# KhutornoyYaroslav/vcm-ts

Hardware: AMD Instinct MI355X
Metric: encoded frames/sec at 1920x1080 GOP-32 (higher is better)
Workload: dtype f32 (fp16x3 split-MFMA, fp32 accumulate)

## Files before the change

include/dcvc_hip.h:

```cpp
#ifndef DCVC_HIP_H
#define DCVC_HIP_H

#include <stdint.h>

#ifdef __cplusplus
extern "C" {
#endif

#define DCVC_OK 0
#define DCVC_E_ARG (-1)
#define DCVC_E_LAUNCH (-2)
#define DCVC_E_RANGE (-3)

#define DCVC_STATUS_ACT_SATURATED 1

#define DCVC_MAX_SEG 3

#define DCVC_PREC_FP32 0
#define DCVC_PREC_FP16X3 1

typedef struct {
    const float *ptr;
    int32_t C;
    int32_t cs;
} dcvc_seg;

typedef struct {
    dcvc_seg seg[DCVC_MAX_SEG];
    int32_t nseg;
    int32_t N, Hin, Win;
    int32_t in_act;
    float in_slope;
    const float *wpack;
    const float *bpack;
    int32_t ks;
    int32_t stride;
    int32_t Cout;
    int32_t Cout_pad;
    float *out;
    int32_t out_cs;
    int32_t out_act;
    float out_slope;
    int32_t pixel_shuffle;
    const float *res;
    int32_t res_cs;
    const float *res_gate;
    const float *res2;
    int32_t res2_cs;
    int32_t precision;
    int32_t *status;
    float *chan_partial;
    int32_t tile_row0;
    int32_t tile_rows;
    int32_t pair_taps;
} dcvc_conv_args;

int32_t dcvc_conv_tile_rows(int32_t ks, int32_t stride);

int32_t dcvc_conv_chan_partial_parts(int32_t ks, int32_t stride, int32_t Hout, int32_t Wout);
int dcvc_channel_mean_finish(const float *chan_partial, int32_t parts, int32_t row_stride, float *mean, int32_t N,
                             int32_t C, int32_t HW, void *stream);

int64_t dcvc_conv_pack_size(int32_t Cout, int32_t ks, int32_t nseg, const int32_t *seg_C, int32_t *cout_pad);

int dcvc_conv_pack_weights(const float *w, const float *b, int32_t Cout, int32_t ks, int32_t nseg,
                           const int32_t *seg_C, int32_t pixel_shuffle, int32_t precision, float *wpack,
                           float *bpack);

int64_t dcvc_conv_pack_size_paired(int32_t Cout, int32_t Cin, int32_t *cout_pad);
int dcvc_conv_pack_weights_paired(const float *w, const float *b, int32_t Cout, int32_t Cin, float *wpack, float *bpack);

int dcvc_conv2d(const dcvc_conv_args *a, void *stream);

int64_t dcvc_conv_small_pack_bytes(int32_t Cout, int32_t ks, int32_t nseg, const int32_t *seg_C);
int dcvc_conv_small_pack_weights(const float *w, const float *b, int32_t Cout, int32_t ks, int32_t nseg,
                                 const int32_t *seg_C, void *wpack, float *bpack);
int dcvc_conv2d_small(const dcvc_conv_args *a, void *stream);

int64_t dcvc_conv_k32_pack_bytes(int32_t Cout, int32_t ks, int32_t nseg, const int32_t *seg_C, int32_t *cout_pad);
int dcvc_conv_k32_pack_weights(const float *w, const float *b, int32_t Cout, int32_t ks, int32_t nseg,
                               const int32_t *seg_C, int32_t pixel_shuffle, void *wpack, float *bpack);
int dcvc_conv2d_k32(const dcvc_conv_args *a, void *stream);
int dcvc_conv_k32_set_waves(int32_t waves);

int dcvc_warp(const float *src, int32_t src_cs, const float *flow, int32_t flow_cs, float *out, int32_t out_cs,
              int32_t N, int32_t H, int32_t W, int32_t C, void *stream);
int dcvc_up2(const float *src, int32_t src_cs, float *out, int32_t out_cs, float *out2, int32_t out2_cs,
             int32_t N, int32_t H, int32_t W, int32_t C, float scale, void *stream);
int dcvc_down2(const float *src, int32_t src_cs, float *out, int32_t out_cs, int32_t N, int32_t H, int32_t W,
               int32_t C, float scale, int32_t avgpool_order, void *stream);
int dcvc_maxpool2(const float *src, int32_t src_cs, float *out, int32_t out_cs, int32_t N, int32_t H, int32_t W,
                  int32_t C, void *stream);
int dcvc_copy_channels(const float *src, int32_t src_cs, float *out, int32_t out_cs, int64_t npix, int32_t C,
                       void *stream);
int dcvc_nchw_to_nhwc(const float *src, float *out, int32_t out_cs, int32_t N, int32_t C, int32_t H, int32_t W,
                      void *stream);
int dcvc_nhwc_to_nchw(const float *src, int32_t src_cs, float *out, int32_t N, int32_t C, int32_t H, int32_t W,
                      int32_t clamp01, void *stream);

int dcvc_channel_mean(const float *src, int32_t src_cs, float *mean, float *scratch, int32_t N, int32_t HW,
                      int32_t C, void *stream);
int dcvc_se_gate(const float *mean, const float *w1, const float *w2, float *gate, int32_t N, int32_t C,
                 int32_t Cr, void *stream);

int dcvc_scale_channels(const float *src, int32_t src_cs, float *out, int32_t out_cs, const float *q_basic,
                        const float *q_scale, int32_t mode, int32_t N, int32_t HW, int32_t C, void *stream);
int dcvc_scale_channels_map(const float *src, int32_t src_cs, float *out, int32_t out_cs, const float *q_basic,
                            const float *q_scale, int32_t mode, int32_t N, int32_t HW, int32_t C, const float *q_map,
                            int32_t H, int32_t W, void *stream);
int dcvc_round_symbols(const float *z, int32_t z_cs, float *z_hat, int32_t zh_cs, int32_t *sym, int32_t N,
                       int32_t H, int32_t W, int32_t C, void *stream);
int dcvc_symbols_to_nhwc(const int32_t *sym, float *out, int32_t out_cs, int32_t N, int32_t H, int32_t W,
                         int32_t C, void *stream);

typedef struct {
    const float *y;
    int32_t y_cs;
    const float *fusion;
    int32_t fusion_cs;
    const float *spatial;
    int32_t spatial_cs;
    float *params;
    int32_t params_cs;
    float *y_hat;
    float *y_q;
    float *y_res;
    float *scales_hat;
    int32_t *sym;
    int32_t *idx;
    float *out;
    int32_t out_cs;
    const float *q_basic;
    const float *q_scale;
    int32_t N, H, W, C;
    int32_t step;
    const float *idx_edges;
    const float *forced_q;
    const float *q_map;
} dcvc_dual_prior_args;

int dcvc_scale_indexes(const float *scales, int32_t *idx, int64_t n, const float *idx_edges, void *stream);

int dcvc_dual_prior_enc(const dcvc_dual_prior_args *a, void *stream);
int dcvc_dual_prior_dec_index(const dcvc_dual_prior_args *a, void *stream);
int dcvc_dual_prior_dec_apply(const dcvc_dual_prior_args *a, void *stream);

int dcvc_scale_bits(const float *y_q, const float *scales_hat, float *out, float *scratch, int32_t kind, int32_t N,
                    int64_t per_sample, void *stream);
int dcvc_factorized_bits(const float *z_hat, int32_t z_cs, const float *params, float *out, float *scratch, int32_t N,
                         int32_t HW, int32_t C, void *stream);
int dcvc_sq_err(const float *a, int32_t a_cs, const float *b, int32_t b_cs, float *out, float *scratch, int32_t N,
                int32_t HW, int32_t C, void *stream);

int32_t dcvc_cdf_table_cols(void);
int dcvc_build_scale_cdfs(const float *scales, int32_t n_scales, int32_t kind, int32_t *cdf, int32_t *sizes,
                          int32_t *offsets, void *stream);
int dcvc_build_factorized_cdfs(const float *params, int32_t C, int32_t *cdf, int32_t *sizes, int32_t *offsets, void *stream);

const char *dcvc_hip_version(void);

#ifdef __cplusplus
}
#endif
#endif
```

vcm_ts_amd/csrc/conv_mfma.hip:

```cpp
#include <hip/hip_runtime.h>
#include <stdint.h>
#include <stdlib.h>
#include <string.h>
#include <vector>

#include "dcvc_hip.h"
#include "kernel_common.h"

namespace {

constexpr int LDK = 20;


struct ConvK {
    const float *seg_ptr[DCVC_MAX_SEG];
    int seg_C[DCVC_MAX_SEG];
    int seg_cs[DCVC_MAX_SEG];
    int nseg;
    int Hin, Win, Hout, Wout;
    int in_act;
    float in_slope;
    const float *wpack;
    const float *bpack;
    int Cout, Cout_pad;
    float *out;
    int out_cs;
    int out_act;
    float out_slope;
    int ps;
    const float *res;
    int res_cs;
    const float *res_gate;
    const float *res2;
    int res2_cs;
    int vec_epi;
    int *status;
    float *chan_partial;
    int ntx;
    int ty0, nty;
    int band_rows;
};

inline long dev_env_long(const char *name, long dflt) {
    const char *dev = getenv("DCVC_DEV");
    if (!dev || strcmp(dev, "1") != 0) return dflt;
    const char *v = getenv(name);
    return v ? atol(v) : dflt;
}


template <int KS, int S, int RPW, int NT, bool SPLIT, bool PAIR = false>
__global__ __launch_bounds__(256, 2) void conv_mfma(const ConvK a) {
    static_assert(!PAIR || (KS == 7 && S == 1 && SPLIT), "tap pairing is built for the 7x7 split-fp16 layers");
    constexpr int BH = 4 * RPW, BW = 32, BN = 32 * NT;
    constexpr int PH = (BH - 1) * S + KS, PW = (BW - 1) * S + KS, PAD = KS / 2;
    constexpr int T = PAIR ? KS * 4 : KS * KS;
    constexpr int TPS = PAIR ? 4 : (KS == 3 && S == 1) ? 9 : KS;
    constexpr int NST = T / TPS;
    constexpr int EPI_LD = BN + 4;
    constexpr int LDS_MAIN = PH * PW * LDK + TPS * 4 * BN * 4, LDS_EPI = 4 * 32 * EPI_LD, LDS_RED = 4 * BN;
    __shared__ __attribute__((aligned(16))) float lds[LDS_MAIN > LDS_EPI + LDS_RED ? LDS_MAIN : LDS_EPI + LDS_RED];
    float *patch = lds;
    float *wl = lds + PH * PW * LDK;

    const int tid = threadIdx.x, lane = tid & 63, wave = tid >> 6;
    const int nbn = a.Cout_pad / BN;
    const int nb = blockIdx.x % nbn, tx = blockIdx.x / nbn;
    if (tx >= a.ntx) return;
    const int ty = blockIdx.y + a.ty0;
    const int x0 = tx * BW, y0 = ty * BH, n0 = nb * BN, img = blockIdx.z;

    f32x16 acc[RPW][NT];
#pragma unroll
    for (int m = 0; m < RPW; ++m)
#pragma unroll
        for (int n = 0; n < NT; ++n)
#pragma unroll
            for (int r = 0; r < 16; ++r) acc[m][n][r] = 0.f;

    const int a_base = ((wave * RPW * S) * PW + (lane & 31) * S) * LDK + (lane >> 5) * 4;
    const int b_base = ((lane >> 5) * BN + (lane & 31)) * 4;

    constexpr int NP = (PH * PW * 4 + 255) / 256, NW = (TPS * 4 * BN + 255) / 256;
    f32x4 rp[NP], rw[NW];
    struct Cursor {
        int s, c0, cg, st;
    };
    auto advance = [&](Cursor &k) {
        if (++k.st == NST) {
            k.st = 0;
            ++k.cg;
            k.c0 += MFMA_KC;
            if (k.c0 >= a.seg_C[k.s]) {
                ++k.s;
                k.c0 = 0;
            }
        }
    };
    int poff[NP];
    unsigned inpic = 0;
#pragma unroll
    for (int u = 0; u < NP; ++u) {
        const int i = tid + u * 256;
        const int p = i >> 2;
        const int py = p / PW, px = p - py * PW + (PAIR ? (i & 3) >> 1 : 0);
        const int gy = y0 * S - PAD + py, gx = x0 * S - PAD + px;
        const bool ok = i < PH * PW * 4 && gy >= 0 && gy < a.Hin && gx >= 0 && gx < a.Win;
        poff[u] = ok ? gy * a.Win + gx : 0;
        inpic |= (ok ? 1u : 0u) << u;
    }
    auto load_patch = [&](const Cursor &k) {
        const int C = a.seg_C[k.s], cs = a.seg_cs[k.s];
        const float *sp = a.seg_ptr[k.s] + (size_t)img * a.Hin * a.Win * cs;
        const int c = PAIR ? (tid & 1) * 4 : k.c0 + (tid & 3) * 4;
        const int cc = c < C ? c : 0;
#pragma unroll
        for (int u = 0; u < NP; ++u) rp[u] = *(const f32x4 *)(sp + (size_t)poff[u] * cs + cc);
    };
    auto store_patch = [&](const Cursor &k) {
        const int C = a.seg_C[k.s];
#pragma unroll
        for (int u = 0; u < NP; ++u) {
            const int i = tid + u * 256;
            if (i < PH * PW * 4) {
                const int c = PAIR ? (i & 1) * 4 : k.c0 + (i & 3) * 4;
                f32x4 v = ((inpic >> u) & 1u) && c < C ? rp[u] : (f32x4){0.f, 0.f, 0.f, 0.f};
                if (c + 3 >= C) {
                    if (c + 1 >= C) v[1] = 0.f;
                    if (c + 2 >= C) v[2] = 0.f;
                    v[3] = 0.f;
                }
                if (a.in_act) {
                    v[0] = act(v[0], a.in_slope);
                    v[1] = act(v[1], a.in_slope);
                    v[2] = act(v[2], a.in_slope);
                    v[3] = act(v[3], a.in_slope);
                }
                if (!SPLIT) {
                    *(f32x4 *)&patch[(i >> 2) * LDK + (i & 3) * 4] = v;
                } else {
                    f32x4 sv = v * ACT_SCALE;
#pragma unroll
                    for (int e = 0; e < 4; ++e) sv[e] = __builtin_amdgcn_fmed3f(sv[e], -F16_MAX, F16_MAX);
                    const f16x4 hi = __builtin_convertvector(sv, f16x4);
                    const f16x4 lo = __builtin_convertvector(sv - __builtin_convertvector(hi, f32x4), f16x4);
                    _Float16 *rec = (_Float16 *)&patch[(i >> 2) * LDK];
                    *(f16x4 *)&rec[(i & 3) * 4] = hi;
                    *(f16x4 *)&rec[16 + (i & 3) * 4] = lo;
                }
            }
        }
    };
    auto load_w = [&](const Cursor &k) {
        const float *wsrc = a.wpack + ((size_t)(k.cg * T + k.st * TPS) * 4) * a.Cout_pad * 4 + (size_t)n0 * 4;
#pragma unroll
        for (int u = 0; u < NW; ++u) {
            const int i = tid + u * 256;
            const int row = i / BN, col = i - row * BN;
            if (i < TPS * 4 * BN) rw[u] = *(const f32x4 *)(wsrc + ((size_t)row * a.Cout_pad + col) * 4);
        }
    };
    auto store_w = [&]() {
#pragma unroll
        for (int u = 0; u < NW; ++u) {
            const int i = tid + u * 256;
            if (i < TPS * 4 * BN) *(f32x4 *)&wl[i * 4] = rw[u];
        }
    };

    Cursor cur = {0, 0, 0, 0};
    load_patch(cur);
    load_w(cur);
    while (cur.s < a.nseg) {
        __syncthreads();
        if (cur.st == 0) store_patch(cur);
        store_w();
        __syncthreads();
        Cursor nxt = cur;
        advance(nxt);
        if (nxt.s < a.nseg) {
            if (nxt.st == 0) load_patch(nxt);
            load_w(nxt);
        }
        const int a_st = (TPS == T) ? 0 : cur.st * PW * LDK;
#pragma unroll
        for (int tt = 0; tt < TPS; ++tt) {
            const int ky = (TPS == T) ? tt / KS : 0, kx = PAIR ? 2 * tt : (TPS == T) ? tt % KS : tt;
            if (!SPLIT) {
#pragma unroll
                for (int k2 = 0; k2 < 2; ++k2) {
                    f32x4 af[RPW], bf[NT];
#pragma unroll
                    for (int m = 0; m < RPW; ++m)
                        af[m] = *(const f32x4 *)&patch[a_base + a_st + ((m * S + ky) * PW + kx) * LDK + k2 * 8];
#pragma unroll
                    for (int n = 0; n < NT; ++n)
                        bf[n] = *(const f32x4 *)&wl[b_base + ((tt * 4 + k2 * 2) * BN + n * 32) * 4];
#pragma unroll
                    for (int j = 0; j < 4; ++j)
#pragma unroll
                        for (int m = 0; m < RPW; ++m)
#pragma unroll
                            for (int n = 0; n < NT; ++n)
                                acc[m][n] = __builtin_amdgcn_mfma_f32_32x32x2f32(af[m][j], bf[n][j], acc[m][n], 0, 0, 0);
                }
            } else {
                f16x8 ah[RPW], al[RPW], bh[NT], bl[NT];
#pragma unroll
                for (int m = 0; m < RPW; ++m) {
                    const float *rec = &patch[a_base + a_st + ((m * S + ky) * PW + kx) * LDK];
                    ah[m] = *(const f16x8 *)rec;
                    al[m] = *(const f16x8 *)(rec + 8);
                }
#pragma unroll
                for (int n = 0; n < NT; ++n) {
                    bh[n] = *(const f16x8 *)&wl[b_base + ((tt * 4) * BN + n * 32) * 4];
                    bl[n] = *(const f16x8 *)&wl[b_base + ((tt * 4 + 2) * BN + n * 32) * 4];
                }
#pragma unroll
                for (int m = 0; m < RPW; ++m)
#pragma unroll
                    for (int n = 0; n < NT; ++n) {
                        acc[m][n] = __builtin_amdgcn_mfma_f32_32x32x16_f16(ah[m], bh[n], acc[m][n], 0, 0, 0);
                        acc[m][n] = __builtin_amdgcn_mfma_f32_32x32x16_f16(ah[m], bl[n], acc[m][n], 0, 0, 0);
                        acc[m][n] = __builtin_amdgcn_mfma_f32_32x32x16_f16(al[m], bh[n], acc[m][n], 0, 0, 0);
                    }
            }
        }
        cur = nxt;
    }

    const int col = lane & 31, hh = lane >> 5;
    const int Cq = a.Cout >> 2;
    const int Cfin = a.ps ? Cq : a.Cout;
    const int Ho = a.ps ? a.Hout * 2 : a.Hout, Wo = a.ps ? a.Wout * 2 : a.Wout;
    const float inv_scale = SPLIT ? 1.f / (ACT_SCALE * WGT_SCALE) : 1.f;
    float vmax = 0.f;
    if (a.vec_epi) {
        constexpr int LPP = BN / 4, PPI = 64 / LPP, NIT = 32 / PPI;
        float *epi = lds + wave * 32 * EPI_LD;
        const int c4 = (lane % LPP) * 4, pl = lane / LPP;
        const int ch = n0 + c4;
        const bool ch_ok = ch < a.Cout;
        int dy = 0, dx = 0, cf = ch;
        if (a.ps) {
            const int sub = ch / Cq;
            cf = ch - sub * Cq;
            dy = sub >> 1;
            dx = sub & 1;
        }
        f32x4 bias = {0.f, 0.f, 0.f, 0.f}, gate = {1.f, 1.f, 1.f, 1.f};
        if (ch_ok) {
            bias = *(const f32x4 *)&a.bpack[ch];
            if (a.res_gate) gate = *(const f32x4 *)&a.res_gate[(size_t)img * Cfin + cf];
        }
        __syncthreads();
        size_t pix[RPW][NIT];
        bool ok[RPW][NIT];
        f32x4 rv[RPW][NIT], rv2[RPW][NIT];
        f32x4 csum = {0.f, 0.f, 0.f, 0.f};
#pragma unroll
        for (int m = 0; m < RPW; ++m) {
            const int oy = y0 + wave * RPW + m;
#pragma unroll
            for (int it = 0; it < NIT; ++it) {
                const int ox = x0 + it * PPI + pl;
                ok[m][it] = ch_ok && oy < a.Hout && ox < a.Wout;
                pix[m][it] = a.ps ? ((size_t)(img * Ho + 2 * oy + dy) * Wo + 2 * ox + dx) : ((size_t)(img * Ho + oy) * Wo + ox);
                rv[m][it] = (f32x4){0.f, 0.f, 0.f, 0.f};
                rv2[m][it] = (f32x4){0.f, 0.f, 0.f, 0.f};
                if (ok[m][it] && a.res) rv[m][it] = *(const f32x4 *)&a.res[pix[m][it] * a.res_cs + cf];
                if (ok[m][it] && a.res2) rv2[m][it] = *(const f32x4 *)&a.res2[pix[m][it] * a.res2_cs + cf];
            }
        }
#pragma unroll
        for (int m = 0; m < RPW; ++m) {
#pragma unroll
            for (int n = 0; n < NT; ++n)
#pragma unroll
                for (int r = 0; r < 16; ++r)
                    epi[((r & 3) + 8 * (r >> 2) + 4 * hh) * EPI_LD + n * 32 + col] = acc[m][n][r];
            asm volatile("s_waitcnt lgkmcnt(0)" ::: "memory");
#pragma unroll
            for (int it = 0; it < NIT; ++it) {
                f32x4 v = *(const f32x4 *)&epi[(it * PPI + pl) * EPI_LD + c4];
                v = v * inv_scale + bias;
                if (a.out_act == 1) {
                    v[0] = act(v[0], a.out_slope);
                    v[1] = act(v[1], a.out_slope);
                    v[2] = act(v[2], a.out_slope);
                    v[3] = act(v[3], a.out_slope);
                } else if (a.out_act == 2) {
#pragma unroll
                    for (int e = 0; e < 4; ++e) v[e] = fminf(fmaxf(v[e], 0.f), 1.f);
                }
                if (a.out_act == 3) {
#pragma unroll
                    for (int e = 0; e < 4; ++e) {
                        const float mk = rv2[m][it][e] > 0.f ? 1.f : a.out_slope;
                        v[e] = a.res ? __builtin_fmaf(v[e], mk, rv[m][it][e]) : v[e] * mk;
                    }
                } else {
                    if (a.res) {
                        if (a.res_gate) {
#pragma unroll
                            for (int e = 0; e < 4; ++e) v[e] = __builtin_fmaf(rv[m][it][e], gate[e], v[e]);
                        } else {
                            v = v + rv[m][it];
                        }
                    }
                    if (a.res2) v = rv2[m][it] + v;
                }
                if (a.chan_partial && ok[m][it]) csum += v;
                if (a.status && ok[m][it])
                    vmax = fmaxf(vmax, fmaxf(fmaxf(fabsf(v[0]), fabsf(v[1])), fmaxf(fabsf(v[2]), fabsf(v[3]))));
                if (ok[m][it]) *(f32x4 *)&a.out[pix[m][it] * a.out_cs + cf] = v;
            }
            asm volatile("s_waitcnt lgkmcnt(0)" ::: "memory");
        }
        if (a.status && !(vmax <= ACT_LIMIT)) atomicOr(a.status, DCVC_STATUS_ACT_SATURATED);
        if (a.chan_partial) {
#pragma unroll
            for (int off = LPP; off < 64; off <<= 1)
#pragma unroll
                for (int e = 0; e < 4; ++e) csum[e] += __shfl_xor(csum[e], off);
            float *red = lds + LDS_EPI;
            if (lane < LPP) *(f32x4 *)&red[wave * BN + c4] = csum;
            __syncthreads();
            if (tid < BN && n0 + tid < a.Cout_pad) {
                const float s = ((red[tid] + red[BN + tid]) + red[2 * BN + tid]) + red[3 * BN + tid];
                const size_t part = (size_t)img * (a.nty * a.ntx) + (size_t)ty * a.ntx + tx;
                a.chan_partial[part * a.Cout_pad + n0 + tid] = s;
            }
        }
        return;
    }
#pragma unroll
    for (int m = 0; m < RPW; ++m) {
        const int oy = y0 + wave * RPW + m;
        if (oy >= a.Hout) continue;
#pragma unroll
        for (int n = 0; n < NT; ++n) {
            const int ch = n0 + n * 32 + col;
            if (ch >= a.Cout) continue;
            const float bias = a.bpack[ch];
            int dy = 0, dx = 0, cf = ch;
            if (a.ps) {
                const int sub = ch / Cq;
                cf = ch - sub * Cq;
                dy = sub >> 1;
                dx = sub & 1;
            }
            const float gate = a.res_gate ? a.res_gate[(size_t)img * Cfin + cf] : 1.f;
            float rv[16], rv2[16];
#pragma unroll
            for (int r = 0; r < 16; ++r) {
                const int ox = x0 + (r & 3) + 8 * (r >> 2) + 4 * hh;
                const size_t pix = a.ps ? ((size_t)(img * Ho + 2 * oy + dy) * Wo + 2 * ox + dx)
                                        : ((size_t)(img * Ho + oy) * Wo + ox);
                rv[r] = (a.res && ox < a.Wout) ? a.res[pix * a.res_cs + cf] : 0.f;
                rv2[r] = (a.res2 && ox < a.Wout) ? a.res2[pix * a.res2_cs + cf] : 0.f;
            }
#pragma unroll
            for (int r = 0; r < 16; ++r) {
                const int ox = x0 + (r & 3) + 8 * (r >> 2) + 4 * hh;
                if (ox >= a.Wout) continue;
                float v = acc[m][n][r] * inv_scale + bias;
                if (a.out_act == 1) v = act(v, a.out_slope);
                else if (a.out_act == 2) v = fminf(fmaxf(v, 0.f), 1.f);
                const size_t pix = a.ps ? ((size_t)(img * Ho + 2 * oy + dy) * Wo + 2 * ox + dx)
                                        : ((size_t)(img * Ho + oy) * Wo + ox);
                if (a.out_act == 3) {
                    const float mk = rv2[r] > 0.f ? 1.f : a.out_slope;
                    v = a.res ? __builtin_fmaf(v, mk, rv[r]) : v * mk;
                } else {
                    if (a.res) v = a.res_gate ? __builtin_fmaf(rv[r], gate, v) : v + rv[r];
                    if (a.res2) v = rv2[r] + v;
                }
                if (a.status) vmax = fmaxf(vmax, fabsf(v));
                a.out[pix * a.out_cs + cf] = v;
            }
        }
    }
    if (a.status && !(vmax <= ACT_LIMIT)) atomicOr(a.status, DCVC_STATUS_ACT_SATURATED);
}


template <int KS, int S, int RPW, int NT, bool PAIR = false>
int launch(ConvK &k, int N, hipStream_t st, int precision) {
    constexpr int BH = 4 * RPW, BN = 32 * NT;
    k.ntx = (k.Wout + 31) / 32;
    static const bool xcd_pad = dev_env_long("DCVC_XCD_PAD", 0) != 0;
    unsigned gx = (unsigned)(k.ntx * (k.Cout_pad / BN));
    if (xcd_pad && gx >= 8) gx = (gx + 7) & ~7u;
    k.nty = (k.Hout + BH - 1) / BH;
    if (k.ty0 < 0 || k.ty0 >= k.nty) return DCVC_E_ARG;
    const int rows = k.band_rows > 0 ? (k.band_rows < k.nty - k.ty0 ? k.band_rows : k.nty - k.ty0) : k.nty;
    dim3 grid(gx, (unsigned)rows, (unsigned)N);
    if (PAIR)
        hipLaunchKernelGGL((conv_mfma<KS, S, RPW, NT, true, PAIR>), grid, dim3(256), 0, st, k);
    else if (precision == DCVC_PREC_FP16X3)
        hipLaunchKernelGGL((conv_mfma<KS, S, RPW, NT, true>), grid, dim3(256), 0, st, k);
    else
        hipLaunchKernelGGL((conv_mfma<KS, S, RPW, NT, false>), grid, dim3(256), 0, st, k);
    RET_LAUNCH();
}

}

extern "C" int64_t dcvc_conv_pack_size(int32_t Cout, int32_t ks, int32_t nseg, const int32_t *seg_C, int32_t *cout_pad) {
    if (Cout <= 0 || nseg <= 0 || nseg > DCVC_MAX_SEG || (ks != 1 && ks != 3 && ks != 7)) return DCVC_E_ARG;
    int chunks = 0;
    for (int s = 0; s < nseg; ++s) chunks += (seg_C[s] + MFMA_KC - 1) / MFMA_KC;
    const int cp = round_up(Cout, 32);
    if (cout_pad) *cout_pad = cp;
    return (int64_t)chunks * ks * ks * 4 * cp * 4;
}

extern "C" int dcvc_conv_pack_weights(const float *w, const float *b, int32_t Cout, int32_t ks, int32_t nseg,
                                      const int32_t *seg_C, int32_t pixel_shuffle, int32_t precision, float *wpack,
                                      float *bpack) {
    if (precision != DCVC_PREC_FP32 && precision != DCVC_PREC_FP16X3) return DCVC_E_ARG;
    int32_t cp = 0;
    const int64_t total = dcvc_conv_pack_size(Cout, ks, nseg, seg_C, &cp);
    if (total < 0 || (pixel_shuffle && (Cout & 3))) return DCVC_E_ARG;
    const int T = ks * ks;
    int Cin = 0;
    for (int s = 0; s < nseg; ++s) Cin += seg_C[s];
    memset(wpack, 0, (size_t)total * sizeof(float));
    memset(bpack, 0, (size_t)cp * sizeof(float));
    const int Cq = Cout / 4;
    _Float16 *base = (_Float16 *)wpack;
    int cg = 0, cin0 = 0;
    for (int s = 0; s < nseg; ++s) {
        for (int c0 = 0; c0 < seg_C[s]; c0 += MFMA_KC, ++cg) {
            for (int t = 0; t < T; ++t)
                for (int cc = 0; cc < MFMA_KC && c0 + cc < seg_C[s]; ++cc)
                    for (int n = 0; n < Cout; ++n) {
                        const int np = pixel_shuffle ? ps_packed_channel(n, Cq) : n;
                        const float v = w[((size_t)n * Cin + cin0 + c0 + cc) * T + t];
                        if (precision == DCVC_PREC_FP32) {
                            wpack[mfma_wpack_f32(cg, T, t, cc, cp, np)] = v;
                        } else {
                            float sv = v * WGT_SCALE;
                            sv = sv > F16_MAX ? F16_MAX : (sv < -F16_MAX ? -F16_MAX : sv);
                            const SplitF16 p = split_f16(sv);
                            base[mfma_wpack_f16(cg, T, t, cc, cp, np, 0)] = p.hi;
                            base[mfma_wpack_f16(cg, T, t, cc, cp, np, 1)] = p.lo;
                        }
                    }
        }
        cin0 += seg_C[s];
    }
    for (int n = 0; n < Cout; ++n) bpack[pixel_shuffle ? ps_packed_channel(n, Cq) : n] = b ? b[n] : 0.f;
    return DCVC_OK;
}

extern "C" int64_t dcvc_conv_pack_size_paired(int32_t Cout, int32_t Cin, int32_t *cout_pad) {
    if (Cout <= 0 || Cin <= 0 || Cin > 8) return DCVC_E_ARG;
    const int cp = round_up(Cout, 32);
    if (cout_pad) *cout_pad = cp;
    return (int64_t)7 * 4 * 4 * cp * 4;
}

extern "C" int dcvc_conv_pack_weights_paired(const float *w, const float *b, int32_t Cout, int32_t Cin, float *wpack, float *bpack) {
    int32_t cp = 0;
    const int64_t total = dcvc_conv_pack_size_paired(Cout, Cin, &cp);
    if (total < 0 || !w || !wpack || !bpack) return DCVC_E_ARG;
    memset(wpack, 0, (size_t)total * sizeof(float));
    memset(bpack, 0, (size_t)cp * sizeof(float));
    _Float16 *base = (_Float16 *)wpack;
    bool clamped = false;
    for (int ky = 0; ky < 7; ++ky)
        for (int kx = 0; kx < 7; ++kx) {
            const int step = ky * 4 + (kx >> 1), h = kx & 1;
            for (int c = 0; c < Cin; ++c)
                for (int n = 0; n < Cout; ++n) {
                    float sv = w[((size_t)n * Cin + c) * 49 + ky * 7 + kx] * WGT_SCALE;
                    if (!(fabsf(sv) <= F16_MAX)) { clamped = true; sv = sv > 0.f ? F16_MAX : -F16_MAX; }
                    const SplitF16 p = split_f16(sv);
                    base[mfma_wpack_f16(0, 28, step, 8 * h + c, cp, n, 0)] = p.hi;
                    base[mfma_wpack_f16(0, 28, step, 8 * h + c, cp, n, 1)] = p.lo;
                }
        }
    for (int n = 0; n < Cout; ++n) bpack[n] = b ? b[n] : 0.f;
    return clamped ? DCVC_E_RANGE : DCVC_OK;
}

static int tile_rows(int ks, int stride) { return stride == 2 ? 4 : 8; }

extern "C" int32_t dcvc_conv_tile_rows(int32_t ks, int32_t stride) { return tile_rows(ks, stride); }

extern "C" int32_t dcvc_conv_chan_partial_parts(int32_t ks, int32_t stride, int32_t Hout, int32_t Wout) {
    if (Hout <= 0 || Wout <= 0 || (stride != 1 && stride != 2)) return DCVC_E_ARG;
    const int bh = tile_rows(ks, stride);
    return ((Wout + 31) / 32) * ((Hout + bh - 1) / bh);
}

extern "C" int dcvc_conv2d(const dcvc_conv_args *a, void *stream) {
    if (!conv_args_ok(a)) return DCVC_E_ARG;
    if (a->stride != 1 && a->stride != 2) return DCVC_E_ARG;
    if (a->precision != DCVC_PREC_FP32 && a->precision != DCVC_PREC_FP16X3) return DCVC_E_ARG;
    if (a->Cout_pad % 32 || a->Cout > a->Cout_pad || (a->pixel_shuffle && (a->Cout & 3))) return DCVC_E_ARG;
    if (a->out_act < 0 || a->out_act > 3) return DCVC_E_ARG;
    if (a->out_act == 3 && (!a->res2 || a->res_gate || a->chan_partial || a->pixel_shuffle)) return DCVC_E_ARG;
    ConvK k;
    memset(&k, 0, sizeof(k));
    copy_conv_args_full(k, a);
    k.Hin = a->Hin;
    k.Win = a->Win;
    const int pad = a->ks / 2;
    k.Hout = (a->Hin + 2 * pad - a->ks) / a->stride + 1;
    k.Wout = (a->Win + 2 * pad - a->ks) / a->stride + 1;
    k.vec_epi = vec_epilogue_ok(a);
    if (a->chan_partial && (!k.vec_epi || a->pixel_shuffle)) return DCVC_E_ARG;
    hipStream_t st = (hipStream_t)stream;
    const bool wide = (a->Cout_pad % 64) == 0;
    const int key = a->ks * 10 + a->stride;
    if (a->stride == 1 && !a->pair_taps && !a->chan_partial && a->tile_rows <= 0) {
        const long wgs8 = (long)((k.Wout + 31) / 32) * ((k.Hout + 7) / 8) * (a->Cout_pad / (wide ? 64 : 32)) * a->N;
        static const long rows4_below = dev_env_long("DCVC_ROWS4_WGS", 384);
        if (wgs8 < rows4_below) {
            if (a->ks == 3) return wide ? launch<3, 1, 1, 2>(k, a->N, st, a->precision) : launch<3, 1, 1, 1>(k, a->N, st, a->precision);
            if (a->ks == 7) return wide ? launch<7, 1, 1, 2>(k, a->N, st, a->precision) : launch<7, 1, 1, 1>(k, a->N, st, a->precision);
            if (a->ks == 1) return wide ? launch<1, 1, 1, 2>(k, a->N, st, a->precision) : launch<1, 1, 1, 1>(k, a->N, st, a->precision);
        }
    }
    switch (key) {
        case 11: return wide ? launch<1, 1, 2, 2>(k, a->N, st, a->precision) : launch<1, 1, 2, 1>(k, a->N, st, a->precision);
        case 12: return wide ? launch<1, 2, 1, 2>(k, a->N, st, a->precision) : launch<1, 2, 1, 1>(k, a->N, st, a->precision);
        case 31:
            return wide ? launch<3, 1, 2, 2>(k, a->N, st, a->precision) : launch<3, 1, 2, 1>(k, a->N, st, a->precision);
        case 32: return wide ? launch<3, 2, 1, 2>(k, a->N, st, a->precision) : launch<3, 2, 1, 1>(k, a->N, st, a->precision);
        case 71:
            if (a->pair_taps) {
                if (a->nseg != 1 || a->seg[0].C > 8 || a->precision != DCVC_PREC_FP16X3 || a->pixel_shuffle) return DCVC_E_ARG;
                return wide ? launch<7, 1, 2, 2, true>(k, a->N, st, a->precision) : launch<7, 1, 2, 1, true>(k, a->N, st, a->precision);
            }
            return wide ? launch<7, 1, 2, 2>(k, a->N, st, a->precision) : launch<7, 1, 2, 1>(k, a->N, st, a->precision);
        default: return DCVC_E_ARG;
    }
}
```

vcm_ts_amd/lib.py:

```python
from __future__ import annotations

import ctypes as C
import os

HERE = os.path.dirname(os.path.abspath(__file__))
CSRC = os.path.join(HERE, "csrc")


class LibraryMissing(RuntimeError):
    pass


class KernelError(RuntimeError):
    pass


def _load(name):
    path = os.environ.get("DCVC_HIP_LIB") if name == "libdcvc_hip.so" and os.environ.get("DCVC_HIP_LIB") else \
        os.path.join(CSRC, name)
    if not os.path.exists(path):
        raise LibraryMissing(f"{path} not built; run `make -C {CSRC}` (no CPU fallback exists)")
    return C.CDLL(path)


_rans = None


def rans():
    global _rans
    if _rans is None:
        L = _load("libdcvc_rans.so")
        L.dcvc_rans_encoder_create.restype = C.c_void_p
        L.dcvc_rans_encoder_destroy.argtypes = [C.c_void_p]
        L.dcvc_rans_encoder_reset.argtypes = [C.c_void_p]
        L.dcvc_rans_encoder_encode_with_indexes.argtypes = [C.c_void_p, C.c_void_p, C.c_void_p, C.c_int64, C.c_void_p,
                                                            C.c_int32, C.c_int32, C.c_void_p, C.c_void_p]
        L.dcvc_rans_encoder_flush_bound.argtypes = [C.c_void_p]
        L.dcvc_rans_encoder_flush_bound.restype = C.c_int64
        L.dcvc_rans_encoder_flush.argtypes = [C.c_void_p, C.c_void_p, C.c_int64]
        L.dcvc_rans_encoder_flush.restype = C.c_int64
        L.dcvc_rans_decoder_create.restype = C.c_void_p
        L.dcvc_rans_decoder_destroy.argtypes = [C.c_void_p]
        L.dcvc_rans_decoder_set_stream.argtypes = [C.c_void_p, C.c_char_p, C.c_int64]
        L.dcvc_rans_decoder_decode_stream.argtypes = [C.c_void_p, C.c_void_p, C.c_int64, C.c_void_p, C.c_int32,
                                                      C.c_int32, C.c_void_p, C.c_void_p, C.c_void_p]
        L.dcvc_pmf_to_quantized_cdf.argtypes = [C.c_void_p, C.c_int32, C.c_int32, C.c_void_p]
        _rans = L
    return _rans


class Seg(C.Structure):
    _fields_ = [("ptr", C.c_void_p), ("C", C.c_int32), ("cs", C.c_int32)]


class ConvArgs(C.Structure):
    _fields_ = [
        ("seg", Seg * 3), ("nseg", C.c_int32), ("N", C.c_int32), ("Hin", C.c_int32), ("Win", C.c_int32),
        ("in_act", C.c_int32), ("in_slope", C.c_float), ("wpack", C.c_void_p), ("bpack", C.c_void_p),
        ("ks", C.c_int32), ("stride", C.c_int32), ("Cout", C.c_int32), ("Cout_pad", C.c_int32),
        ("out", C.c_void_p), ("out_cs", C.c_int32), ("out_act", C.c_int32), ("out_slope", C.c_float),
        ("pixel_shuffle", C.c_int32), ("res", C.c_void_p), ("res_cs", C.c_int32), ("res_gate", C.c_void_p),
        ("res2", C.c_void_p), ("res2_cs", C.c_int32), ("precision", C.c_int32), ("status", C.c_void_p),
        ("chan_partial", C.c_void_p), ("tile_row0", C.c_int32), ("tile_rows", C.c_int32), ("pair_taps", C.c_int32),
    ]


class DualPriorArgs(C.Structure):
    _fields_ = [
        ("y", C.c_void_p), ("y_cs", C.c_int32), ("fusion", C.c_void_p), ("fusion_cs", C.c_int32),
        ("spatial", C.c_void_p), ("spatial_cs", C.c_int32), ("params", C.c_void_p), ("params_cs", C.c_int32),
        ("y_hat", C.c_void_p), ("y_q", C.c_void_p), ("y_res", C.c_void_p), ("scales_hat", C.c_void_p),
        ("sym", C.c_void_p), ("idx", C.c_void_p), ("out", C.c_void_p), ("out_cs", C.c_int32),
        ("q_basic", C.c_void_p), ("q_scale", C.c_void_p), ("N", C.c_int32), ("H", C.c_int32), ("W", C.c_int32),
        ("C", C.c_int32), ("step", C.c_int32), ("idx_edges", C.c_void_p), ("forced_q", C.c_void_p),
        ("q_map", C.c_void_p),
    ]


class ConvBwdArgs(C.Structure):
    _fields_ = [
        ("dout", C.c_void_p), ("dout_cs", C.c_int32), ("out", C.c_void_p), ("out_cs", C.c_int32),
        ("res", C.c_void_p), ("res_cs", C.c_int32), ("gate", C.c_void_p), ("res2", C.c_void_p), ("res2_cs", C.c_int32),
        ("dres", C.c_void_p), ("dres_cs", C.c_int32), ("dres2", C.c_void_p), ("dres2_cs", C.c_int32),
        ("dpre", C.c_void_p), ("dpre_cs", C.c_int32), ("zs", C.c_int32), ("Hd", C.c_int32), ("Wd", C.c_int32),
        ("N", C.c_int32), ("Ho", C.c_int32), ("Wo", C.c_int32), ("Cout", C.c_int32), ("pixel_shuffle", C.c_int32),
        ("act", C.c_int32), ("slope", C.c_float),
    ]


class WgradArgs(C.Structure):
    _fields_ = [
        ("x", C.c_void_p), ("x_cs", C.c_int32), ("C", C.c_int32), ("in_act", C.c_int32), ("in_slope", C.c_float),
        ("dpre", C.c_void_p), ("dpre_cs", C.c_int32), ("zs", C.c_int32), ("Hd", C.c_int32), ("Wd", C.c_int32),
        ("N", C.c_int32), ("Hin", C.c_int32), ("Win", C.c_int32), ("Ho", C.c_int32), ("Wo", C.c_int32),
        ("Cout", C.c_int32), ("ks", C.c_int32), ("stride", C.c_int32), ("dw", C.c_void_p), ("Cin_total", C.c_int32),
        ("cin_offset", C.c_int32), ("scratch", C.c_void_p), ("scratch_floats", C.c_int64), ("overwrite", C.c_int32),
        ("db", C.c_void_p), ("precision", C.c_int32),
    ]


class PackJob(C.Structure):
    _fields_ = [
        ("w", C.c_void_p), ("b", C.c_void_p), ("Cout", C.c_int32), ("Cin_total", C.c_int32), ("ks", C.c_int32),
        ("nseg", C.c_int32), ("seg_C", C.c_int32 * 3), ("cin_offset", C.c_int32), ("pixel_shuffle", C.c_int32),
        ("precision", C.c_int32), ("transposed", C.c_int32), ("wpack", C.c_void_p), ("bpack", C.c_void_p),
    ]


class DualPriorBwdArgs(C.Structure):
    _fields_ = [
        ("y", C.c_void_p), ("y_cs", C.c_int32), ("fusion", C.c_void_p), ("fusion_cs", C.c_int32),
        ("y_hat", C.c_void_p), ("dout", C.c_void_p), ("dout_cs", C.c_int32), ("dy_res", C.c_void_p),
        ("dscales_hat", C.c_void_p), ("dparams", C.c_void_p), ("dparams_cs", C.c_int32),
        ("dspatial", C.c_void_p), ("dspatial_cs", C.c_int32), ("dy", C.c_void_p), ("dy_cs", C.c_int32),
        ("dfusion", C.c_void_p), ("dfusion_cs", C.c_int32), ("dq_plane", C.c_void_p),
        ("q_basic", C.c_void_p), ("q_scale", C.c_void_p), ("N", C.c_int32), ("H", C.c_int32), ("W", C.c_int32),
        ("C", C.c_int32), ("step", C.c_int32),
    ]


class ColorCoeffs(C.Structure):
    _fields_ = [(n, C.c_float) for n in ("y_off", "c_off", "y_scale", "c_scale", "crr", "cgb", "cgr", "cbb", "kr", "kg", "kb",
                                         "icb", "icr", "y_range", "c_range")] + \
               [(n, C.c_int32) for n in ("max_code", "bit_depth", "siting", "matrix", "range")]


class RoiBox(C.Structure):
    _fields_ = [(n, C.c_int32) for n in ("x1", "y1", "x2", "y2", "cls")]


class RoiClassRec(C.Structure):
    _fields_ = [("border", C.c_int32), ("shrink", C.c_int32), ("feather", C.c_float * 64)]


PRECISIONS = {"fp32": 0, "fp16x3": 1}

_hip = None
i32, i64, f32, vp = C.c_int32, C.c_int64, C.c_float, C.c_void_p

_SIGS = {
    "dcvc_conv2d": [C.POINTER(ConvArgs), vp],
    "dcvc_conv_pack_weights": [vp, vp, i32, i32, i32, vp, i32, i32, vp, vp],
    "dcvc_conv_pack_weights_paired": [vp, vp, i32, i32, vp, vp],
    "dcvc_conv2d_small": [C.POINTER(ConvArgs), vp],
    "dcvc_conv_small_pack_weights": [vp, vp, i32, i32, i32, vp, vp, vp],
    "dcvc_conv2d_k32": [C.POINTER(ConvArgs), vp],
    "dcvc_conv_k32_pack_weights": [vp, vp, i32, i32, i32, vp, i32, vp, vp],
    "dcvc_conv_k32_set_waves": [i32],
    "dcvc_warp": [vp, i32, vp, i32, vp, i32, i32, i32, i32, i32, vp],
    "dcvc_up2": [vp, i32, vp, i32, vp, i32, i32, i32, i32, i32, f32, vp],
    "dcvc_down2": [vp, i32, vp, i32, i32, i32, i32, i32, f32, i32, vp],
    "dcvc_maxpool2": [vp, i32, vp, i32, i32, i32, i32, i32, vp],
    "dcvc_copy_channels": [vp, i32, vp, i32, i64, i32, vp],
    "dcvc_nchw_to_nhwc": [vp, vp, i32, i32, i32, i32, i32, vp],
    "dcvc_nhwc_to_nchw": [vp, i32, vp, i32, i32, i32, i32, i32, vp],
    "dcvc_channel_mean": [vp, i32, vp, vp, i32, i32, i32, vp],
    "dcvc_se_gate": [vp, vp, vp, vp, i32, i32, i32, vp],
    "dcvc_channel_mean_finish": [vp, i32, i32, vp, i32, i32, i32, vp],
    "dcvc_scale_channels": [vp, i32, vp, i32, vp, vp, i32, i32, i32, i32, vp],
    "dcvc_scale_channels_map": [vp, i32, vp, i32, vp, vp, i32, i32, i32, i32, vp, i32, i32, vp],
    "dcvc_round_symbols": [vp, i32, vp, i32, vp, i32, i32, i32, i32, vp],
    "dcvc_symbols_to_nhwc": [vp, vp, i32, i32, i32, i32, i32, vp],
    "dcvc_scale_indexes": [vp, vp, i64, vp, vp],
    "dcvc_dual_prior_enc": [C.POINTER(DualPriorArgs), vp],
    "dcvc_dual_prior_dec_index": [C.POINTER(DualPriorArgs), vp],
    "dcvc_dual_prior_dec_apply": [C.POINTER(DualPriorArgs), vp],
    "dcvc_build_scale_cdfs": [vp, i32, i32, vp, vp, vp, vp],
    "dcvc_build_factorized_cdfs": [vp, i32, vp, vp, vp, vp],
    "dcvc_scale_bits": [vp, vp, vp, vp, i32, i32, i64, vp],
    "dcvc_factorized_bits": [vp, i32, vp, vp, vp, i32, i32, i32, vp],
    "dcvc_sq_err": [vp, i32, vp, i32, vp, vp, i32, i32, i32, vp],
    "dcvc_conv_pack_weights_dev": [vp, vp, i32, i32, i32, i32, vp, i32, i32, i32, i32, vp, vp, vp],
    "dcvc_pack_plan_create": [C.POINTER(PackJob), i32, C.POINTER(C.c_void_p)],
    "dcvc_pack_plan_run": [vp, vp],
    "dcvc_pack_plan_destroy": [vp],
    "dcvc_conv_bwd_prologue": [C.POINTER(ConvBwdArgs), vp],
    "dcvc_conv_wgrad": [C.POINTER(WgradArgs), vp],
    "dcvc_channel_dot": [vp, i32, vp, i32, vp, vp, i32, i32, i32, i32, i32, vp],
    "dcvc_mask_accumulate": [vp, i32, vp, i32, f32, vp, i32, i64, i32, vp],
    "dcvc_add_planes": [vp, i32, vp, i32, vp, i32, i64, i32, vp],
    "dcvc_warp_bwd": [vp, i32, vp, i32, vp, i32, vp, i32, vp, i32, i32, i32, i32, i32, vp, vp],
    "dcvc_up2_bwd": [vp, i32, vp, i32, i32, i32, i32, i32, f32, vp],
    "dcvc_down2_bwd": [vp, i32, vp, i32, i32, i32, i32, i32, f32, vp],
    "dcvc_maxpool2_bwd": [vp, i32, vp, i32, vp, i32, i32, i32, i32, i32, vp],
    "dcvc_se_bwd": [vp, vp, vp, vp, vp, vp, vp, vp, i32, i32, i32, vp],
    "dcvc_add_channel_vec": [vp, i32, vp, f32, i32, i32, i32, vp],
    "dcvc_scale_channels_bwd": [vp, i32, vp, i32, vp, vp, i32, i32, i32, i32, vp],
    "dcvc_q_finish": [vp, vp, vp, vp, vp, vp, i32, i32, vp],
    "dcvc_dual_prior_bwd": [C.POINTER(DualPriorBwdArgs), vp],
    "dcvc_scale_bits_bwd": [vp, vp, vp, vp, vp, i32, i32, i64, vp],
    "dcvc_factorized_bits_bwd": [vp, i32, vp, vp, vp, i32, vp, i32, i32, i32, vp],
    "dcvc_sq_err_bwd": [vp, i32, vp, i32, vp, vp, i32, i32, i32, i32, vp],
    "dcvc_drans_encode": [vp, vp, i32, i32, i64, vp, i32, i32, vp, vp, i32, vp, i64, vp, i64, vp, vp, vp, vp],
    "dcvc_drans_decode": [vp, i64, vp, vp, vp, i32, i32, i64, vp, i32, i32, vp, vp, vp, i32, vp, vp, vp],
    "dcvc_drans_build_lut": [vp, i32, i32, vp, vp],
    "dcvc_ms_ssim": [vp, vp, i32, i32, i32, i32, i32, i64, i32, i64, f32, i32, vp, vp, vp, vp, vp],
    "dcvc_ms_ssim_grad": [vp, vp, i32, i32, i32, i32, i32, i64, i32, i64, f32, i32, vp, vp, vp, vp],
    "dcvc_color_coeffs": [i32, i32, i32, i32, vp],
    "dcvc_yuv420_to_rgb": [vp, vp, vp, i32, i32, i32, i32, vp, vp, i32, i32, i32, i64, i32, vp],
    "dcvc_rgb_to_yuv420": [vp, i32, i32, i32, i64, vp, vp, vp, vp, i32, i32, vp, vp, vp, i32, i32, vp, vp],
    "dcvc_roi_residual": [vp, i32, i64, vp, i32, i64, i32, i32, vp, vp, i32, vp, i64, i64, i32, i32, i32, i32, vp],
    "dcvc_roi_fuse": [vp, i32, i64, vp, i64, i64, i32, i32, i32, i32, i32, i32, vp, vp, i32, vp, i32, vp, i32, i64, vp],
    "dcvc_roi_sse": [vp, i32, i64, vp, i32, i64, i32, i32, vp, vp, i32, vp, i32, vp, vp],
    "dcvc_roi_qmap": [i32, i32, vp, vp, i32, i32, vp, i32, vp, vp],
    "dcvc_roil_cells": [i32, i32, vp, i32, vp, vp, i32],
    "dcvc_roil_check": [vp, i64, vp, i32],
    "dcvc_roil_encode": [vp, i32, i64, vp, i32, i64, i32, i32, vp, vp, i32, i32, vp, i32, vp, vp, i64, vp, vp],
    "dcvc_roil_decode": [vp, vp, i64, i32, i32, vp, vp, i32, vp, vp, i64, i64, i32, i32, i32, i32, vp, vp],
    "dcvc_scene_hist": [vp, i32, i64, i32, i32, vp, vp],
    "dcvc_bits_map_scale": [vp, vp, vp, vp, vp, i32, i32, vp, vp, vp, i32, i32, i32, i32, vp, vp],
    "dcvc_bits_map_factorized": [vp, vp, i32, i32, vp, vp, vp, i32, i32, i32, i32, vp, vp],
    "dcvc_bits_regions": [vp, vp, i32, vp, i32, i32, i32, vp, vp],
    "dcvc_bits_sweep_scale": [vp, vp, vp, vp, i32, vp, i32, i32, vp, vp, vp, i32, i32, i32, i32, vp, vp],
    "dcvc_hash_pixels": [vp, i32, i64, i32, i32, vp, vp, vp],
    "dcvc_hash_f32": [vp, i32, i64, i32, i32, i32, vp, vp, vp],
    "dcvc_scale_planes": [vp, i32, i64, vp, i32, i64, i32, i32, i32, i32, i32, vp, vp, vp, vp, i32, vp, vp, vp, vp, i32, vp],
    "dcvc_aq_activity": [vp, i32, i64, i32, i32, vp, vp, vp],
    "dcvc_aq_map": [vp, vp, i32, i32, vp, vp, vp, vp, vp],
    "dcvc_motion_step": [vp, i32, i64, i32, i32, vp, i32, i32, i32, i32, vp, vp],
    "dcvc_tnr_step": [vp, i32, i64, vp, i32, i64, vp, i32, i64, i32, i32, vp, i32, vp, vp, vp],
}

METRICS_SYMBOLS = ["dcvc_ms_ssim", "dcvc_ms_ssim_grad", "dcvc_ms_ssim_workspace_bytes"]
COLOR_SYMBOLS = ["dcvc_color_coeffs", "dcvc_yuv420_to_rgb", "dcvc_rgb_to_yuv420"]
ROI_SYMBOLS = ["dcvc_roi_residual", "dcvc_roi_fuse", "dcvc_roi_sse", "dcvc_roi_qmap"]
ROIL_SYMBOLS = ["dcvc_roil_cells", "dcvc_roil_check", "dcvc_roil_encode", "dcvc_roil_decode"]
SCENE_SYMBOLS = ["dcvc_scene_hist"]
BITS_SYMBOLS = ["dcvc_bits_map_scale", "dcvc_bits_map_factorized", "dcvc_bits_regions",
                "dcvc_bits_sweep_scale"]
HASH_SYMBOLS = ["dcvc_hash_pixels", "dcvc_hash_f32"]
HASH_CONSTANTS = ["dcvc_hash_chunk_bytes", "dcvc_hash_block_bytes", "dcvc_hash_scratch_bytes"]
SCALE_SYMBOLS = ["dcvc_scale_planes"]
AQ_SYMBOLS = ["dcvc_aq_activity", "dcvc_aq_map"]
MOTION_SYMBOLS = ["dcvc_motion_step"]
TNR_SYMBOLS = ["dcvc_tnr_step"]
HIP_SYMBOLS = sorted([s for s in _SIGS if s not in METRICS_SYMBOLS + COLOR_SYMBOLS + ROI_SYMBOLS + ROIL_SYMBOLS + SCENE_SYMBOLS + BITS_SYMBOLS + HASH_SYMBOLS + SCALE_SYMBOLS + AQ_SYMBOLS + MOTION_SYMBOLS + TNR_SYMBOLS] +
                     ["dcvc_cdf_table_cols", "dcvc_conv_pack_size", "dcvc_conv_pack_size_paired", "dcvc_conv_small_pack_bytes", "dcvc_conv_k32_pack_bytes", "dcvc_conv_tile_rows", "dcvc_conv_chan_partial_parts", "dcvc_hip_version", "dcvc_conv_wgrad_scratch_min",
                      "dcvc_drans_default_lanes", "dcvc_drans_scratch_words"])
RANS_SYMBOLS = [
    "dcvc_rans_encoder_create", "dcvc_rans_encoder_destroy", "dcvc_rans_encoder_reset",
    "dcvc_rans_encoder_encode_with_indexes", "dcvc_rans_encoder_flush_bound", "dcvc_rans_encoder_flush",
    "dcvc_rans_decoder_create", "dcvc_rans_decoder_destroy", "dcvc_rans_decoder_set_stream",
    "dcvc_rans_decoder_decode_stream", "dcvc_pmf_to_quantized_cdf",
]


def hip():
    global _hip
    if _hip is None:
        L = _load("libdcvc_hip.so")
        for name, sig in _SIGS.items():
            fn = getattr(L, name)
            fn.argtypes = sig
            fn.restype = C.c_int
        L.dcvc_pack_plan_destroy.restype = None
        L.dcvc_conv_pack_size.argtypes = [i32, i32, i32, vp, C.POINTER(i32)]
        L.dcvc_conv_pack_size.restype = i64
        L.dcvc_conv_pack_size_paired.argtypes = [i32, i32, C.POINTER(i32)]
        L.dcvc_conv_pack_size_paired.restype = i64
        L.dcvc_cdf_table_cols.argtypes = []
        L.dcvc_cdf_table_cols.restype = i32
        L.dcvc_conv_chan_partial_parts.argtypes = [i32, i32, i32, i32]
        L.dcvc_conv_chan_partial_parts.restype = i32
        L.dcvc_conv_small_pack_bytes.argtypes = [i32, i32, i32, vp]
        L.dcvc_conv_small_pack_bytes.restype = i64
        L.dcvc_conv_tile_rows.argtypes = [i32, i32]
        L.dcvc_conv_tile_rows.restype = i32
        L.dcvc_conv_k32_pack_bytes.argtypes = [i32, i32, i32, vp, C.POINTER(i32)]
        L.dcvc_conv_k32_pack_bytes.restype = i64
        L.dcvc_hip_version.restype = C.c_char_p
        L.dcvc_conv_wgrad_scratch_min.argtypes = [i32, i32, i32]
        L.dcvc_conv_wgrad_scratch_min.restype = i64
        L.dcvc_drans_default_lanes.argtypes = [i64]
        L.dcvc_drans_default_lanes.restype = i32
        L.dcvc_drans_scratch_words.argtypes = [i64, i32]
        L.dcvc_drans_scratch_words.restype = i64
        L.dcvc_ms_ssim_workspace_bytes.argtypes = [i32, i32, i32, i32, i32]
        L.dcvc_ms_ssim_workspace_bytes.restype = i64
        _hip = L
    return _hip


def hash_constant(name):
    return int(i32.in_dll(hip(), name).value)


def check(code, what):
    if code != 0:
        raise KernelError(f"{what} failed with status {code}")
```

Baseline: 42.48.

## Add lookahead variant of MFMA conv main loop for 7x7 and strided 3x3

Adds an AHEAD template variant of the conv_mfma kernel that restructures the K loop into per-chunk straight-line steps. The next chunk's input patch is prefetched during the first step of the current chunk, and weights one step ahead. Weight loads drop their bounds check by redirecting the overhanging float4 into the slab. This is meant to hide global load latency behind MFMA work for 7x7 and stride-2 3x3 layers. The variant is the default (g_lookahead=2) and can be switched back through a new setter, at the cost of more register pressure and extra template instantiations.

```diff
diff --git a/include/dcvc_hip.h b/include/dcvc_hip.h
--- a/include/dcvc_hip.h
+++ b/include/dcvc_hip.h
@@ -71,6 +71,7 @@
 int dcvc_conv_pack_weights_paired(const float *w, const float *b, int32_t Cout, int32_t Cin, float *wpack, float *bpack);
 
 int dcvc_conv2d(const dcvc_conv_args *a, void *stream);
+int dcvc_conv_set_lookahead(int32_t mode);
 
 int64_t dcvc_conv_small_pack_bytes(int32_t Cout, int32_t ks, int32_t nseg, const int32_t *seg_C);
 int dcvc_conv_small_pack_weights(const float *w, const float *b, int32_t Cout, int32_t ks, int32_t nseg,
diff --git a/vcm_ts_amd/csrc/conv_mfma.hip b/vcm_ts_amd/csrc/conv_mfma.hip
--- a/vcm_ts_amd/csrc/conv_mfma.hip
+++ b/vcm_ts_amd/csrc/conv_mfma.hip
@@ -2,6 +2,7 @@
 #include <stdint.h>
 #include <stdlib.h>
 #include <string.h>
+#include <type_traits>
 #include <vector>
 
 #include "dcvc_hip.h"
@@ -41,6 +42,8 @@
     int band_rows;
 };
 
+int g_lookahead = 2;
+
 inline long dev_env_long(const char *name, long dflt) {
     const char *dev = getenv("DCVC_DEV");
     if (!dev || strcmp(dev, "1") != 0) return dflt;
@@ -49,7 +52,7 @@
 }
 
 
-template <int KS, int S, int RPW, int NT, bool SPLIT, bool PAIR = false>
+template <int KS, int S, int RPW, int NT, bool SPLIT, bool PAIR = false, bool AHEAD = false>
 __global__ __launch_bounds__(256, 2) void conv_mfma(const ConvK a) {
     static_assert(!PAIR || (KS == 7 && S == 1 && SPLIT), "tap pairing is built for the 7x7 split-fp16 layers");
     constexpr int BH = 4 * RPW, BW = 32, BN = 32 * NT;
@@ -82,6 +85,7 @@
     const int b_base = ((lane >> 5) * BN + (lane & 31)) * 4;
 
     constexpr int NP = (PH * PW * 4 + 255) / 256, NW = (TPS * 4 * BN + 255) / 256;
+    static_assert(!AHEAD || NST >= 3, "AHEAD: two straight-line steps and a loop over the rest of a chunk");
     f32x4 rp[NP], rw[NW];
     struct Cursor {
         int s, c0, cg, st;
@@ -151,38 +155,30 @@
             }
         }
     };
+    constexpr int W_OVER = NW * 256 - TPS * 4 * BN;
+    static_assert(!AHEAD || TPS * 4 * BN >= W_OVER, "the doubled float4 must lie inside the slab");
+    auto w_slot = [&](const int u) {
+        const int i = tid + u * 256;
+        return AHEAD && W_OVER > 0 && u == NW - 1 && i >= TPS * 4 * BN ? i - W_OVER : i;
+    };
     auto load_w = [&](const Cursor &k) {
         const float *wsrc = a.wpack + ((size_t)(k.cg * T + k.st * TPS) * 4) * a.Cout_pad * 4 + (size_t)n0 * 4;
 #pragma unroll
         for (int u = 0; u < NW; ++u) {
-            const int i = tid + u * 256;
+            const int i = w_slot(u);
             const int row = i / BN, col = i - row * BN;
-            if (i < TPS * 4 * BN) rw[u] = *(const f32x4 *)(wsrc + ((size_t)row * a.Cout_pad + col) * 4);
+            if (AHEAD || i < TPS * 4 * BN) rw[u] = *(const f32x4 *)(wsrc + ((size_t)row * a.Cout_pad + col) * 4);
         }
     };
     auto store_w = [&]() {
 #pragma unroll
         for (int u = 0; u < NW; ++u) {
-            const int i = tid + u * 256;
-            if (i < TPS * 4 * BN) *(f32x4 *)&wl[i * 4] = rw[u];
-        }
-    };
-
-    Cursor cur = {0, 0, 0, 0};
-    load_patch(cur);
-    load_w(cur);
-    while (cur.s < a.nseg) {
-        __syncthreads();
-        if (cur.st == 0) store_patch(cur);
-        store_w();
-        __syncthreads();
-        Cursor nxt = cur;
-        advance(nxt);
-        if (nxt.s < a.nseg) {
-            if (nxt.st == 0) load_patch(nxt);
-            load_w(nxt);
-        }
-        const int a_st = (TPS == T) ? 0 : cur.st * PW * LDK;
+            const int i = w_slot(u);
+            if (AHEAD || i < TPS * 4 * BN) *(f32x4 *)&wl[i * 4] = rw[u];
+        }
+    };
+    auto mfma_step = [&](const int st) {
+        const int a_st = (TPS == T) ? 0 : st * PW * LDK;
 #pragma unroll
         for (int tt = 0; tt < TPS; ++tt) {
             const int ky = (TPS == T) ? tt / KS : 0, kx = PAIR ? 2 * tt : (TPS == T) ? tt % KS : tt;
@@ -227,7 +223,63 @@
                     }
             }
         }
-        cur = nxt;
+    };
+
+    Cursor cur = {0, 0, 0, 0};
+    if constexpr (AHEAD) {
+        auto chunk = [&](auto more, const Cursor &nc) {
+            constexpr bool MORE = decltype(more)::value;
+            __syncthreads();
+            store_patch(cur);
+            store_w();
+            __syncthreads();
+            advance(cur);
+            load_w(cur);
+            if (MORE) load_patch(nc);
+            mfma_step(0);
+            auto row_step = [&](const int st) {
+                __syncthreads();
+                store_w();
+                __syncthreads();
+                if (st + 1 < NST) {
+                    advance(cur);
+                    load_w(cur);
+                } else if (MORE) {
+                    load_w(nc);
+                }
+                mfma_step(st);
+            };
+            row_step(1);
+            for (int st = 2; st < NST; ++st) row_step(st);
+        };
+        load_patch(cur);
+        load_w(cur);
+        for (;;) {
+            Cursor nc = cur;
+            nc.st = NST - 1;
+            advance(nc);
+            if (nc.s >= a.nseg) break;
+            chunk(std::true_type{}, nc);
+            cur = nc;
+        }
+        chunk(std::false_type{}, cur);
+    } else {
+        load_patch(cur);
+        load_w(cur);
+        while (cur.s < a.nseg) {
+            __syncthreads();
+            if (cur.st == 0) store_patch(cur);
+            store_w();
+            __syncthreads();
+            Cursor nxt = cur;
+            advance(nxt);
+            if (nxt.s < a.nseg) {
+                if (nxt.st == 0) load_patch(nxt);
+                load_w(nxt);
+            }
+            mfma_step(cur.st);
+            cur = nxt;
+        }
     }
 
     const int col = lane & 31, hh = lane >> 5;
@@ -397,6 +449,18 @@
     if (k.ty0 < 0 || k.ty0 >= k.nty) return DCVC_E_ARG;
     const int rows = k.band_rows > 0 ? (k.band_rows < k.nty - k.ty0 ? k.band_rows : k.nty - k.ty0) : k.nty;
     dim3 grid(gx, (unsigned)rows, (unsigned)N);
+    constexpr bool HAS_AHEAD = (KS == 3 && S == 2) || KS == 7;
+    if constexpr (HAS_AHEAD) {
+        if (g_lookahead == 2) {
+            if (PAIR)
+                hipLaunchKernelGGL((conv_mfma<KS, S, RPW, NT, true, PAIR, true>), grid, dim3(256), 0, st, k);
+            else if (precision == DCVC_PREC_FP16X3)
+                hipLaunchKernelGGL((conv_mfma<KS, S, RPW, NT, true, false, true>), grid, dim3(256), 0, st, k);
+            else
+                hipLaunchKernelGGL((conv_mfma<KS, S, RPW, NT, false, false, !(KS == 7 && RPW == 2 && NT == 2)>), grid, dim3(256), 0, st, k);
+            RET_LAUNCH();
+        }
+    }
     if (PAIR)
         hipLaunchKernelGGL((conv_mfma<KS, S, RPW, NT, true, PAIR>), grid, dim3(256), 0, st, k);
     else if (precision == DCVC_PREC_FP16X3)
@@ -497,6 +561,12 @@
     return ((Wout + 31) / 32) * ((Hout + bh - 1) / bh);
 }
 
+extern "C" int dcvc_conv_set_lookahead(int32_t mode) {
+    if (mode != 1 && mode != 2) return DCVC_E_ARG;
+    g_lookahead = mode;
+    return DCVC_OK;
+}
+
 extern "C" int dcvc_conv2d(const dcvc_conv_args *a, void *stream) {
     if (!conv_args_ok(a)) return DCVC_E_ARG;
     if (a->stride != 1 && a->stride != 2) return DCVC_E_ARG;
diff --git a/vcm_ts_amd/lib.py b/vcm_ts_amd/lib.py
--- a/vcm_ts_amd/lib.py
+++ b/vcm_ts_amd/lib.py
@@ -142,6 +142,7 @@
     "dcvc_conv2d": [C.POINTER(ConvArgs), vp],
     "dcvc_conv_pack_weights": [vp, vp, i32, i32, i32, vp, i32, i32, vp, vp],
     "dcvc_conv_pack_weights_paired": [vp, vp, i32, i32, vp, vp],
+    "dcvc_conv_set_lookahead": [i32],
     "dcvc_conv2d_small": [C.POINTER(ConvArgs), vp],
     "dcvc_conv_small_pack_weights": [vp, vp, i32, i32, i32, vp, vp, vp],
     "dcvc_conv2d_k32": [C.POINTER(ConvArgs), vp],
```

Measured after the change: 43.11, median of 6. +1.5%, better.
